# mhsitu/welding_robot

Measured on AMD Instinct MI355X. Metric: acs_generations_per_sec, higher is better.
Workload: dtype f32

## Files before the change

### include/weldacs.h

```cpp
#ifndef WELDACS_H
#define WELDACS_H
#include <stddef.h>
#include <stdint.h>

#ifdef __cplusplus
extern "C" {
#endif

typedef enum {
    WA_OK = 0,
    WA_ERR_ARG = 1,
    WA_ERR_DEVICE = 2,
    WA_ERR_ALLOC = 3,
    WA_ERR_FILE = 4,
    WA_ERR_FORMAT = 5,
    WA_ERR_POINT = 6,
    WA_ERR_CAPACITY = 7,
    WA_ERR_STATE = 8
} wa_status;

typedef struct wa_ctx wa_ctx;
typedef struct wa_grid wa_grid;
typedef struct wa_acs wa_acs;
typedef struct wa_traj wa_traj;
// ... 78 lines not shown
int wa_acs_read_pheromone(wa_acs *s, int32_t slot, float *out );
int wa_acs_read_ants(wa_acs *s, int32_t slot, int32_t *colony, float *L, int32_t *len, int32_t cap);
int wa_acs_read_ant_path(wa_acs *s, int32_t slot, int32_t ant, int32_t *ids, int32_t cap, int32_t *len);
int wa_acs_last_params(wa_acs *s, int32_t slot, int32_t *colony, float *lambda, float *Q);

enum { WA_K_WALK = 0, WA_K_RANK = 1, WA_K_EVAPORATE = 2, WA_K_DEPOSIT = 3, WA_K_COUNT = 4 };
int wa_acs_profile(wa_acs *s, int32_t enable, int32_t sample_every);
int wa_acs_walk_info(const wa_acs *s, int32_t out[4]);
int wa_acs_profile_read(wa_acs *s, double ms[WA_K_COUNT], int64_t launches[WA_K_COUNT]);
int wa_acs_debug_counters(wa_acs *s, uint64_t out16[16], int32_t reset);
int wa_acs_straggler_counters(wa_acs *s, int32_t slot, uint64_t *handed_over, uint64_t *resumed, int32_t reset);
int wa_acs_set_stragglers(wa_acs *s, int32_t generations);
int wa_acs_converged_info(wa_acs *s, int32_t slot, uint64_t out[4]);
int wa_acs_converged_host_info(wa_acs *s, uint64_t out[4]);
int wa_acs_converged_owed_info(wa_acs *s, uint64_t out[5]);
int wa_acs_evaporate(wa_acs *s, int32_t slot, float rho, int32_t repeats);

#define WA_COMM_ID_BYTES 128
typedef struct wa_comm wa_comm;
int wa_comm_unique_id(uint8_t id_out[WA_COMM_ID_BYTES]);
int wa_comm_create(wa_ctx *ctx, int32_t rank, int32_t world, const uint8_t id[WA_COMM_ID_BYTES], wa_comm **out);
void wa_comm_destroy(wa_comm *c);
int wa_comm_info(const wa_comm *c, int32_t *rank, int32_t *world);
int wa_comm_abort(wa_comm *c);
int wa_comm_stats(wa_comm *c, int64_t out[5]);
int wa_acs_allreduce_best(wa_acs *s, wa_comm *c, int32_t gen0, int32_t count);
int wa_comm_read_best(wa_comm *c, int32_t gen0, int32_t count, float *out);
int wa_comm_read_best_owner(wa_comm *c, int32_t gen0, int32_t count, float *cost, int32_t *owner_rank, int32_t *owner_slot);
int wa_comm_pack_best_key(float cost, int32_t rank, int32_t slot, uint64_t *key);
int wa_comm_unpack_best_key(uint64_t key, float *cost, int32_t *rank, int32_t *slot);
// ... 289 lines not shown
```

### welding_robot_amd/_lib.py

```python
import ctypes as C
import os

HERE = os.path.dirname(os.path.abspath(__file__))
LIB_PATH = os.environ.get("WELDACS_LIB") or os.path.join(HERE, "lib", "libweldacs.so")

WA_OK = 0
STATUS = {0: "WA_OK", 1: "WA_ERR_ARG", 2: "WA_ERR_DEVICE", 3: "WA_ERR_ALLOC", 4: "WA_ERR_FILE",
          5: "WA_ERR_FORMAT", 6: "WA_ERR_POINT", 7: "WA_ERR_CAPACITY", 8: "WA_ERR_STATE"}
RNG_REF, RNG_DEV = 0, 1
K_WALK, K_RANK, K_EVAPORATE, K_DEPOSIT, K_COUNT = 0, 1, 2, 3, 4


class AcsParams(C.Structure):
    _fields_ = [("alpha", C.c_int32), ("beta", C.c_float), ("rho", C.c_float), ("pheromone_0", C.c_float),
                ("max_iteration", C.c_int32), ("predict", C.c_float), ("fixed_colony", C.c_int32),
                ("rng_mode", C.c_int32), ("seed", C.c_uint64)]


class GtspParams(C.Structure):
    _fields_ = [("rng_mode", C.c_int32), ("seed", C.c_uint64), ("stream", C.c_uint32),
                ("max_iterations", C.c_int32)]


WA_D2_NONE = 0x7fffffff
# ... 153 lines not shown
    "wa_acs_result_batch": (C.c_int, [_V, _I, _P, _P, _P, _I64]),
    "wa_acs_result_batch_choices": (C.c_int, [_V, _I, _P, _P, _P, _P, _I64]),
    "wa_acs_trace": (C.c_int, [_V, _I, _P, _P, _P, _P, _P, _P]),
    "wa_acs_export_trace": (C.c_int, [_V, _V, _I, _I]),
    "wa_acs_read_pheromone": (C.c_int, [_V, _I, _P]),
    "wa_acs_read_ants": (C.c_int, [_V, _I, _P, _P, _P, _I]),
    "wa_acs_read_ant_path": (C.c_int, [_V, _I, _I, _P, _I, _P]),
    "wa_acs_last_params": (C.c_int, [_V, _I, _P, _P, _P]),
    "wa_acs_profile": (C.c_int, [_V, _I, _I]),
    "wa_acs_profile_read": (C.c_int, [_V, _P, _P]),
    "wa_acs_debug_counters": (C.c_int, [_V, _P, _I]),
    "wa_acs_straggler_counters": (C.c_int, [_V, _I, _P, _P, _I]),
    "wa_acs_converged_info": (C.c_int, [_V, _I, _P]),
    "wa_acs_converged_host_info": (C.c_int, [_V, _P]),
    "wa_acs_converged_owed_info": (C.c_int, [_V, _P]),
    "wa_acs_set_stragglers": (C.c_int, [_V, _I]),
    "wa_acs_walk_info": (C.c_int, [_V, _P]),
    "wa_acs_evaporate": (C.c_int, [_V, _I, _F, _I]),
    "wa_comm_unique_id": (C.c_int, [_P]),
    "wa_comm_create": (C.c_int, [_V, _I, _I, _P, C.POINTER(_V)]),
    "wa_comm_destroy": (None, [_V]),
    "wa_comm_info": (C.c_int, [_V, _P, _P]),
    "wa_comm_abort": (C.c_int, [_V]),
    "wa_comm_stats": (C.c_int, [_V, _P]),
    "wa_acs_allreduce_best": (C.c_int, [_V, _V, _I, _I]),
    "wa_comm_read_best": (C.c_int, [_V, _I, _I, _P]),
    "wa_comm_read_best_owner": (C.c_int, [_V, _I, _I, _P, _P, _P]),
    "wa_comm_pack_best_key": (C.c_int, [_F, _I, _I, _P]),
    "wa_comm_unpack_best_key": (C.c_int, [C.c_uint64, _P, _P, _P]),
    "wa_comm_allgather_costs": (C.c_int, [_V, _I, _P, _P, _I, _P]),
# ... 95 lines not shown
```

### welding_robot_amd/api.py

```python
import atexit
import ctypes as C
import weakref

import numpy as np

from . import _lib as L
from ._lib import AcsParams, GtspParams, RNG_DEV, RNG_REF, WA_COST_MAX, WA_D2_NONE, WA_DIST_NONE, WA_HOPS_NONE, WeldacsError


RETIME_Q = 1 << 30


def _ptr(a):
    return a.ctypes.data if a is not None else None


_live_contexts = weakref.WeakSet()


@atexit.register
def _close_live_contexts():
    for c in list(_live_contexts):
        try:
            c.close()
# ... 500 lines not shown

    def converged_info(self, slot=0):
        out = (C.c_uint64 * 4)()
        self.ctx.check(self.ctx.lib.wa_acs_converged_info(self.h, slot, out))
        return dict(enqueued=int(out[0]), whole=int(out[1]), cut=int(out[2]), generations=int(out[3]))

    def converged_host_info(self):
        out = (C.c_uint64 * 4)()
        self.ctx.check(self.ctx.lib.wa_acs_converged_host_info(self.h, out))
        return [int(v) for v in out]

    def converged_owed_info(self):
        out = (C.c_uint64 * 5)()
        self.ctx.check(self.ctx.lib.wa_acs_converged_owed_info(self.h, out))
        return dict(carried=int(out[0]), merged=int(out[1]), fallback=int(out[2]), out_of_place=int(out[3]), in_place=int(out[4]))

    def set_stragglers(self, generations):
        self.ctx.check(self.ctx.lib.wa_acs_set_stragglers(self.h, generations))

    def set_pipeline(self, groups):
        self.ctx.check(self.ctx.lib.wa_acs_set_pipeline(self.h, groups))

    def pipeline_groups(self):
        g = C.c_int32()
        self.ctx.check(self.ctx.lib.wa_acs_pipeline_info(self.h, C.byref(g)))
        return g.value

    def solve(self, params, starts, ends, streams=None):
        starts, ends, streams = self._arrs(starts, ends, streams)
        self.n_active = len(starts)
# ... 661 lines not shown
```

### welding_robot_amd/csrc/acs_converged.hpp

```cpp
#pragma once

#define WA_CONV_CHECK_WAVES 4
#define WA_CONV_ADV_WAVES 4
#define WA_CONV_THREADS ((WA_CONV_CHECK_WAVES + WA_CONV_ADV_WAVES) * 64)
#define WA_CONV_BLOCKS 64
#define WA_CONV_BLOCKS_MAX 256
#define WA_CONV_MAX_WINDOW 64
#define WA_CONV_NODE_CAP 1024
#define WA_CONV_NODE_LDS 128
#define WA_CONV_SNAP 14

struct WaConvHdr {
    uint32_t rem;
    uint32_t ticket;
    int32_t pending;
    int32_t carried;
    unsigned long long whole, cut, gens;
    unsigned long long pad2_[3];
};
static_assert(WA_CONV_SNAP == 14, "wa_table_rows strides the owed records by 14 floats");
static_assert(sizeof(WaConvHdr) == 64, "the snapshots start 64 bytes into the block");

__device__ __forceinline__ WaConvHdr *wa_conv_hdr(const WaAcsDev &D, int32_t slot) { return reinterpret_cast<WaConvHdr *>(D.conv + (int64_t)slot * D.conv_stride); }
__device__ __forceinline__ float *wa_conv_snap(const WaAcsDev &D, int32_t slot, int32_t t)
{
    return reinterpret_cast<float *>(D.conv + (int64_t)slot * D.conv_stride + sizeof(WaConvHdr)) + (int64_t)t * D.conv_nodes * WA_CONV_SNAP;
}
__device__ __forceinline__ int32_t wa_conv_pending(const WaAcsDev &D, int32_t slot) { return wa_conv_hdr(D, slot)->pending; }
__device__ __forceinline__ bool wa_conv_carried(const WaAcsDev &D, int32_t slot) { return wa_conv_hdr(D, slot)->carried != 0; }
__device__ __forceinline__ const float *wa_conv_owed_records(const WaAcsDev &D, int32_t slot) { return wa_conv_snap(D, slot, wa_conv_pending(D, slot) - 1); }
#define WA_CONV_CARRIED 0x80u

__device__ __forceinline__ void wa_conv_flush_rows(const WaAcsDev &D, int32_t slot, int32_t first, int32_t step, bool rows_only)
{
    const int32_t blen = D.ctl[slot].best_len, j = wa_conv_pending(D, slot);
    if (j < 1) return;
    const float *snap = wa_conv_snap(D, slot, j - 1);
    const int32_t *bpath = D.bestpath + (int64_t)slot * D.path_cap;
    float *pher = D.pher + (int64_t)slot * D.pher_stride;
    float *T = D.rtab + (int64_t)slot * D.path_cap * 8;
    for (int32_t x = first; x < blen * WA_CONV_SNAP; x += step) {
        const int32_t i = x / WA_CONV_SNAP, q = x - i * WA_CONV_SNAP;
        const float v = snap[x];
        if (q < 6) { if (!rows_only) pher[(int64_t)(bpath[i] & (int32_t)WA_ID_MASK) * 6 + q] = v; }
// ... 264 lines not shown
```

### welding_robot_amd/csrc/acs_dev.hpp

```cpp
#pragma once

#define WA_GEN_SPEC 0x40000000
#define WA_GEN_OWED 0x20000000
#define WA_GEN_FLAGS (WA_GEN_SPEC | WA_GEN_OWED)

struct WaAcsDev {
    WaDims d;
    const float *cx, *cy, *cz;
    const uint8_t *occ;
    float *pher, *heur;
    unsigned long long *mask;
    uint8_t *mask8;
    uint32_t *bestmark;
    int32_t *bestpos;
    uint8_t *besttabu;
    int32_t *bestpath;
    float *rtab;
    int32_t *paths;
    float *antL;
    int32_t *antLen;
    int32_t *antRep;
    int32_t *perm;
    float *depA;
    float *sortk;
// ... 230 lines not shown
```

### welding_robot_amd/csrc/acs_update.hpp

```cpp
#pragma once
struct WaRec { float k; int32_t t; };
__device__ inline void ss_push_heap(WaRec *first, long hole, long top, WaRec value)
{
    long parent = (hole - 1) / 2;
    while (hole > top && first[parent].k < value.k) {
        first[hole] = first[parent];
        hole = parent;
        parent = (hole - 1) / 2;
    }
    first[hole] = value;
}
__device__ inline void ss_adjust_heap(WaRec *first, long hole, long len, WaRec value)
{
    const long top = hole;
    long child = hole;
    while (child < (len - 1) / 2) {
        child = 2 * (child + 1);
        if (first[child].k < first[child - 1].k) child--;
        first[hole] = first[child];
        hole = child;
    }
    if ((len & 1) == 0 && child == (len - 2) / 2) {
        child = 2 * (child + 1);
        first[hole] = first[child - 1];
// ... 203 lines not shown
        c.bestL = bestL;
        c.dep_lambda = lambda;
        c.dep_Q = Q;
        c.dep_bestL = bestL;
        c.n_dep = s_ndep;
        c.gen = gen + 1;
        c.rep_mask = 0;
        wa_next_params(c, R, (gen + 1) & 1);
        *ctl = c;
    }
}

typedef float wa_v4f __attribute__((ext_vector_type(4)));
__device__ __forceinline__ int32_t wa_conv_pending(const WaAcsDev &D, int32_t slot);
__device__ __forceinline__ bool wa_conv_carried(const WaAcsDev &D, int32_t slot);
template <int NT>
__device__ __forceinline__ wa_v4f wa_sweep_ld(const wa_v4f *p) { return (NT & 1) ? __builtin_nontemporal_load(p) : *p; }
template <int NT>
__device__ __forceinline__ void wa_sweep_st(wa_v4f *p, wa_v4f v)
{
    if (NT & 2) __builtin_nontemporal_store(v, p);
    else *p = v;
}
template <int NT>
__device__ __forceinline__ void wa_sweep_body_nt(const float *src, float *dst, int64_t n_floats, float rho, int32_t ebx, int32_t E, int32_t reps)
{
    const wa_v4f *s4 = reinterpret_cast<const wa_v4f *>(src);
    wa_v4f *d4 = reinterpret_cast<wa_v4f *>(dst);
    const int64_t n4 = n_floats >> 2;
    const int64_t gsz = (int64_t)E * blockDim.x;
// ... 24 lines not shown
    default: wa_sweep_body_nt<3>(src, dst, n_floats, rho, ebx, E, reps); break;
    }
}

#define WA_LEN_OF(x) ((x) & 0x3fffffff)
template <bool SPARSE, int NB>
__global__ __launch_bounds__(256) void k_evap_rank_mark(WaAcsDev D, WaRun R, const float *src_base,
                                                        float *dst_base, int32_t E, int32_t gen, int32_t MB, int32_t split_log2, int32_t lazy_period,
                                                        int32_t sweep_nt, int32_t rank_cap)
{
    extern __shared__ unsigned long long wa_rank_lds[];
    const int32_t slot = blockIdx.y, tid = threadIdx.x;
    const int32_t gflags = gen & WA_GEN_FLAGS;
    gen &= ~WA_GEN_FLAGS;
    if ((gflags & WA_GEN_SPEC) && gen + 1 != D.ctl[slot].spec_until) return;
    if (gen < D.ctl[slot].spec_until) {
        if (!SPARSE && NB == 6 && gen + 1 == D.ctl[slot].spec_until && (int32_t)blockIdx.x >= MB) {
            if ((gflags & WA_GEN_OWED) && wa_conv_carried(D, slot)) return;
            const int32_t j = wa_conv_pending(D, slot);
            float *to = dst_base + (int64_t)slot * D.pher_stride;
            wa_sweep_body((j & 1) ? src_base + (int64_t)slot * D.pher_stride : to, to, (int64_t)NB * D.d.n, R.rho, (int32_t)blockIdx.x - MB, E, sweep_nt, j);
        }
        return;
    }
    if ((int32_t)blockIdx.x >= MB) {
#ifdef WA_TEST_KNOBS
        if (sweep_nt & 0x100) return;
#endif
        if (!SPARSE) {
            float *to = dst_base + (int64_t)slot * D.pher_stride;
// ... 453 lines not shown
```

### welding_robot_amd/csrc/acs_walk.hpp

```cpp
#pragma once
struct WaTabu {
    int32_t *tab;
    uint32_t mask, shift;
    uint32_t *bits;
    bool spilled;
    bool t16 = false;
    uint32_t kmul = 0;
    int32_t hl = 0;
    int32_t ovf_dw = 0;
};
#define WA_T16_EMPTY 0xFFFFu
#define WA_T16_SENTINEL 0xFFFEu
#define WA_T16_MAXD 13u
__device__ __forceinline__ uint32_t wa_t16_idx(const WaTabu &t, uint32_t tt) { return tt >> (32 - t.hl); }
__device__ __forceinline__ uint32_t wa_t16_cmp(const WaTabu &t, uint32_t tt) { return (tt >> (16 - t.hl)) & 0xFFF0u; }
__device__ __forceinline__ bool tabu_has(const WaTabu &t, int32_t key)
{
    if (t.spilled) {
        uint32_t w = __hip_atomic_load(&t.bits[(uint32_t)key >> 5], __ATOMIC_RELAXED, __HIP_MEMORY_SCOPE_AGENT);
        return (w >> (key & 31)) & 1u;
    }
    if (t.t16) {
        const volatile uint16_t *tb = reinterpret_cast<const volatile uint16_t *>(t.tab);
        const uint32_t tt = (uint32_t)key * t.kmul, c = wa_t16_cmp(t, tt);
// ... 848 lines not shown
        if (k2 == 0) T[(int64_t)i * 8 + 7] = __int_as_float(i + 1 < blen ? (int32_t)((uint32_t)wn >> WA_K_SHIFT) : -1);
    }
}

__global__ __launch_bounds__(256) void k_replay_table(WaAcsDev D, WaRun R)
{
    const int32_t row0 = (blockIdx.x * blockDim.x + threadIdx.x) >> 4;
    const int32_t *bpath = D.bestpath + (int64_t)blockIdx.y * D.path_cap;
    const int32_t w0 = row0 < D.path_cap ? bpath[row0] : 0, w1 = row0 + 1 < D.path_cap ? bpath[row0 + 1] : 0;
    wa_table_rows(D, R, blockIdx.y, row0, (gridDim.x * blockDim.x) >> 4, false, 0.f, 0, w0, w1);
}

#define WA_TABLE_BLOCKS_MAX 64
__device__ __forceinline__ void wa_conv_flush_rows(const WaAcsDev &D, int32_t slot, int32_t first, int32_t step, bool rows_only);
__device__ __forceinline__ bool wa_conv_carried(const WaAcsDev &D, int32_t slot);
__device__ __forceinline__ const float *wa_conv_owed_records(const WaAcsDev &D, int32_t slot);
__global__ __launch_bounds__(256) void k_apply_table(WaAcsDev D, WaRun R, int32_t split_log2, int32_t table_blocks, int32_t gen)
{
    const int32_t slot = blockIdx.y;
    const int32_t spec_until = D.ctl[slot].spec_until;
    const int32_t gflags = gen & WA_GEN_FLAGS;
    gen &= ~WA_GEN_FLAGS;
    if ((gflags & WA_GEN_SPEC) && gen + 1 != spec_until) return;
    if (gen + 1 < spec_until) return;
    if (D.dcount && blockIdx.x == 0 && threadIdx.x == 0) D.dcount[slot * 2] = D.dcount[slot * 2 + 1];
    if (D.pool_n && blockIdx.x == 0) {
        const WaStrag sg = wa_strag_of(D, slot);
        sg.arr_len[threadIdx.x] = 0xffffffffu;
        if (threadIdx.x == 0) { *sg.arr_n = 0; sg.pool_n[D.ctl[slot].gen & 1] = 0; }
    }
    if (gen < spec_until) {
        if ((int32_t)blockIdx.x < table_blocks)
            wa_conv_flush_rows(D, slot, blockIdx.x * blockDim.x + threadIdx.x, table_blocks * blockDim.x, (gflags & WA_GEN_OWED) && wa_conv_carried(D, slot));
        return;
    }
    if ((int32_t)blockIdx.x < table_blocks) {
        const int32_t lane = threadIdx.x & 63, row0 = (blockIdx.x * blockDim.x + threadIdx.x) >> 4;
        const float dep_lane = lane < D.max_colony ? D.depA[(int64_t)slot * D.max_colony + lane] : 0.f;
// ... 2 lines not shown
        const int32_t n_dep = D.ctl[slot].n_dep;
        wa_table_rows(D, R, slot, row0, (table_blocks * blockDim.x) >> 4, true, dep_lane, n_dep < 64 ? n_dep : 64, w0, w1,
                      (gflags & WA_GEN_OWED) ? wa_conv_owed_records(D, slot) : nullptr);
        return;
    }
    const int32_t ab = (int32_t)blockIdx.x - table_blocks;
    wa_apply_body<6>(D, slot, 0, ab >> split_log2, ab & ((1 << split_log2) - 1), 1 << split_log2, true);
}

template <bool ALPHA1, bool SPARSE, bool WARM = true, bool REJ = true, bool DIRECT = false, bool T16 = false>
__global__ __launch_bounds__(64) void k_walk_dev(WaAcsDev D, WaRun R, int hash_log2, int32_t gen, int32_t walk_flags)
{
    extern __shared__ int32_t lds[];
    const int32_t slot = blockIdx.y, ant = blockIdx.x;
    const WaSlotCtl *c = &D.ctl[slot];
    if (gen < c->spec_until) return;
    const int32_t colony = c->colony[gen & 1];
#ifdef WA_STRAG_TIME
    if (threadIdx.x == 0 && gen < 128) atomicMax(&wa_strag_t[gen * 8 + 0], ~(unsigned long long)wall_clock64());
#endif
    if (!SPARSE && ALPHA1 && D.pool_n && (int32_t)blockIdx.x >= D.max_colony) {
        const int32_t r = (int32_t)blockIdx.x - D.max_colony, pg = (gen - 1) & 1;
        const WaStrag sg = wa_strag_of(D, slot);
        if (gen < 1 || r >= sg.pool_n[pg] || r >= WA_RESUME_MAX) return;
        const int32_t a = sg.pool_rec[(pg * WA_RESUME_MAX + r) * WA_POOL_REC], n0 = sg.pool_rec[(pg * WA_RESUME_MAX + r) * WA_POOL_REC + 1];
        WaAcsDev Dp = D;
        Dp.pher = const_cast<float *>(D.prev_pher);
        const uint64_t key = wa_ctr_antkey(wa_ctr_key(R.seed, c->stream, (uint32_t)(gen - 1)), (uint32_t)a);
        int32_t f0 = 0, b0 = 0, rs0 = 0;
        wa_walk_one<1, true, false, WARM, false, DIRECT, T16>(Dp, R, slot, a, c->start, c->end, key, lds, hash_log2, rs0, f0, b0, &D.ctl[slot].flags, 0, INFINITY, 0.f, 0u,
// ... 175 lines not shown
```

### welding_robot_amd/csrc/host_acs.inc

```
static int acs_drain(wa_acs *s);
void wa_acs_default_params(wa_acs_params *p)
{
    if (!p) return;
    p->alpha = 1;
    p->beta = 0.6f;
    p->rho = 0.8f;
    p->pheromone_0 = 1.f;
    p->max_iteration = 150;
    p->predict = 10.f;
    p->fixed_colony = 0;
    p->rng_mode = WA_RNG_DEV;
    p->seed = 1;
}


static_assert(WA_PLAN_REF_SPEC_LEN == WA_REF_SPEC_LEN && WA_PLAN_REF_SUPER == WA_REF_SUPER && WA_PLAN_RESUME_MAX == WA_RESUME_MAX &&
              WA_PLAN_POOL_REC == WA_POOL_REC && WA_PLAN_ROW26 == WA_ROW26, "acs_plan.hpp and the kernels' headers disagree");
static WaPlanIn acs_plan_in(const wa_grid *grid, int32_t n_slots, int32_t max_colony, int64_t path_capacity, int32_t nb, bool lazy)
{
    int32_t fields0 = n_slots < 4 ? n_slots : 4;
    if (n_slots >= 32) fields0 = n_slots / 8 < 8 ? 8 : (n_slots / 8 > 24 ? 24 : n_slots / 8);
    return WaPlanIn{grid->d.n, grid->d.nxy, n_slots, max_colony, fields0, path_capacity, nb, lazy ? 1 : 0,
                    env_int("WA_MASK_U64", 0), env_int("WA_REPLAY", 1), env_int("WA_REF_SPEC", 1), env_int("WA_STRAGGLERS", 1), env_int("WA_STRAGGLER_SLOTS", 16),
                    (int64_t)sizeof(WaSlotCtl), (int64_t)sizeof(WaGlibcRand)};
// ... 107 lines not shown
    s->hw_queues = env_int("GPU_MAX_HW_QUEUES", 4);
    s->drain_ok = env_int("WA_STRAGGLER_DRAIN", 1) != 0;
    s->sweep_nt_env = env_int("WA_SWEEP_NT", -1);
    s->straggler_gens = env_int("WA_STRAGGLER_GENS", 64);
    s->conv_on = env_int("WA_CONVERGED_RUN", 1) != 0;
    s->conv_window = env_int("WA_CONVERGED_WINDOW", 32);
    if (s->conv_window > WA_CONV_MAX_WINDOW) s->conv_window = WA_CONV_MAX_WINDOW;
    if (s->conv_window < 1) s->conv_on = false;
    s->conv_nodes_env = env_int("WA_CONVERGED_NODES", 0);
    s->conv_blocks = env_int("WA_CONVERGED_BLOCKS", WA_CONV_BLOCKS);
    s->conv_blocks = s->conv_blocks < 1 ? 1 : s->conv_blocks > WA_CONV_BLOCKS_MAX ? WA_CONV_BLOCKS_MAX : s->conv_blocks;
    s->conv_readback = env_int("WA_CONVERGED_READBACK", 1) != 0;
    s->conv_wait_us = env_int("WA_CONVERGED_WAIT_US", 200000);
    s->conv_spec = env_int("WA_CONVERGED_SPECULATE", 1) != 0;
    s->conv_owed = env_int("WA_CONVERGED_OWED", 1) != 0;
    s->conv_enqueued.assign((size_t)n_slots, 0);
    {
        const int64_t n4 = (int64_t)nb * n / 4;
        int64_t blocks = n4 <= ((int64_t)8 << 20) ? 4096 : n4 / 555;
        if (blocks > 65536) blocks = 65536;
        s->evap_blocks = env_int("WA_EVAP_BLOCKS", (int)blocks);
    }
    hipError_t e = hipSuccess;
    const bool trace_create = env_int("WA_TRACE_CREATE", 0) != 0;
    const auto t_create0 = std::chrono::steady_clock::now();
    auto since0 = [&]() { return std::chrono::duration<double>(std::chrono::steady_clock::now() - t_create0).count(); };
    bool pools = P.pools;
    for (const WaPlanRow &r : P.rows) {
        if (e || (r.pool && !pools)) continue;
        if (&r == &P.rows[P.heur_row]) { e = (hipError_t)heur_pool_grow(s, &D, (int32_t)P.fields0); continue; }
// ... 338 lines not shown
            else k_heuristic<6><<<hg, 256, 0, ctx->stream>>>(s->D, R.beta, s->d_hlist, s->d_hends);
        }
        he_ = hipGetLastError();
    }
    he_ = he_ ? he_ : hipStreamSynchronize(ctx->stream);
    if (he_ != hipSuccess) {
        for (int32_t f : hlist) { s->heur_end[f] = -1; s->heur_used[f] = 0; }
        s->begun = false;
        return fail(ctx, WA_ERR_DEVICE, "wa_acs_begin: %s", hipGetErrorString(he_));
    }
    s->n_active = n_problems;
    s->begun = true;
    s->gens_enqueued = 0;
    s->conv_until = 0;
    s->conv_prev_whole = false;
    s->conv_owed_flush = s->conv_owed_gen = -1;
    s->ran_before = false;
    return WA_OK;
}

static EvPair *prof_open(wa_acs *s, hipStream_t st, int cls, bool sampled)
{
    if (!sampled) return nullptr;
    EvPair p;
    p.cls = cls;
    if (hipEventCreate(&p.a) != hipSuccess) return nullptr;
    if (hipEventCreate(&p.b) != hipSuccess) { hipEventDestroy(p.a); return nullptr; }
    hipEventRecord(p.a, st);
    s->ev.push_back(p);
    return &s->ev.back();
// ... 137 lines not shown
        if (hipEventCreate(&p.b) == hipSuccess) ev = true;
        else hipEventDestroy(p.a);
    }
    if (ev) {
        if (s->nb == 26) hipExtLaunchKernelGGL((k_evap_rank_mark<false, 26>), grid, dim3(256), rank_lds, G.st, p.a, p.b, 0, G.V, s->R, src, dst, s->evap_blocks, gen, MB, SL, LP, G.sweep_nt, RC);
        else hipExtLaunchKernelGGL((k_evap_rank_mark<false, 6>), grid, dim3(256), rank_lds, G.st, p.a, p.b, 0, G.V, s->R, src, dst, s->evap_blocks, gen, MB, SL, LP, G.sweep_nt, RC);
    } else if (s->nb == 26) {
        k_evap_rank_mark<false, 26><<<grid, 256, rank_lds, G.st>>>(G.V, s->R, src, dst, s->evap_blocks, gen, MB, SL, LP, G.sweep_nt, RC);
    } else {
        k_evap_rank_mark<false, 6><<<grid, 256, rank_lds, G.st>>>(G.V, s->R, src, dst, s->evap_blocks, gen, MB, SL, LP, G.sweep_nt, RC);
    }
    if (ev) s->ev.push_back(p);
}

static void enqueue_generation(wa_acs *s, WaGroupRun &G, int32_t gen, bool last_of_call, bool sampled, bool fused, int32_t chunks,
                               size_t shmem, int32_t P_all, bool owed = false)
{
    wa_ctx *ctx = s->ctx;
    const int32_t P = G.P;
    hipStream_t st = G.st;
    const int64_t off = (int64_t)G.slot0 * s->D.pher_stride;
    float *src = s->pher_buf[G.cur] + off, *dst = s->pher_buf[G.cur ^ (s->lazy ? 0 : 1)] + off;
    G.V.pher = src;
    G.V.prev_pher = s->lazy ? nullptr : s->pher_buf[G.cur ^ 1] + off;
    {
        const int64_t poff = (int64_t)G.slot0 * s->D.max_colony * s->D.path_cap;
        G.V.paths = s->paths_arr[gen & 1] + poff;
        G.V.prev_paths = s->paths_arr[(gen + 1) & 1] + poff;
    }
    EvPair *e = prof_open(s, st, WA_K_WALK, sampled);
    const bool strag = s->D.pool_n != nullptr && fused && s->R.rng_mode == WA_RNG_DEV && s->R.alpha == 1 && gen <= s->straggler_gens;
// ... 12 lines not shown
        }
    } else if (s->R.rng_mode == WA_RNG_DEV) {
        if (s->colony_bound > 0) {
            dim3 wg((unsigned)(strag ? s->D.max_colony + WA_RESUME_MAX : s->colony_bound), (unsigned)P);
            const int walk_flags = s->walk_flags | (hand_over ? 32 : 0);
            const bool warm = s->walk_direct <= 0 && s->tab16_env != 1 && (s->walk_warm < 0 ? (int64_t)s->colony_bound * P_all <= ctx->prop.multiProcessorCount : s->walk_warm != 0);
            const bool rej = (walk_flags & 2) && gen >= ((walk_flags >> 24) & 127);
            const bool direct = !warm && (s->walk_direct < 0 ? walk_direct_rule(s, P_all) : s->walk_direct != 0);
            bool t16 = false;
            if (!warm && !direct && s->R.alpha == 1 && (walk_flags & 1) && s->D.tab16_kmul != 0 && s->id_bits <= s->hash_log2 + 12) {
                int64_t per_cu = 160 * 1024 / (int64_t)shmem;
                if (per_cu > 16) per_cu = 16;
                t16 = s->tab16_env == 1 || (s->tab16_env < 0 && s->id_bits <= 21 && (int64_t)wg.x * P_all > per_cu * ctx->prop.multiProcessorCount);
            }
            const size_t shmem16 = ((size_t)2 << s->hash_log2) + WA_WALK_LDS_EXTRA + (size_t)s->lds_pad;
#define WA_LAUNCH_WALK16(SP, RJ) k_walk_dev<true, SP, false, RJ, false, true><<<wg, 64, shmem16, st>>>(G.V, s->R, s->hash_log2, gen, walk_flags)
#define WA_LAUNCH_WALK(A1, SP, WM, RJ, DR) k_walk_dev<A1, SP, WM, RJ, DR><<<wg, 64, shmem, st>>>(G.V, s->R, s->hash_log2, gen, walk_flags)
            s->last_walk[0] = s->hash_log2; s->last_walk[1] = t16 ? 1 : 0; s->last_walk[2] = (int32_t)(t16 ? shmem16 : shmem); s->last_walk[3] = warm ? 1 : 0;
            if (t16) {
                if (s->lazy) { if (rej) WA_LAUNCH_WALK16(true, true); else WA_LAUNCH_WALK16(true, false); }
                else { if (rej) WA_LAUNCH_WALK16(false, true); else WA_LAUNCH_WALK16(false, false); }
            } else if (s->R.alpha != 1) {
                if (s->lazy) WA_LAUNCH_WALK(false, true, true, true, false); else WA_LAUNCH_WALK(false, false, true, true, false);
            } else if (s->lazy) {
                if (warm) { if (rej) WA_LAUNCH_WALK(true, true, true, true, false); else WA_LAUNCH_WALK(true, true, true, false, false); }
                else if (direct) { if (rej) WA_LAUNCH_WALK(true, true, false, true, true); else WA_LAUNCH_WALK(true, true, false, false, true); }
                else { if (rej) WA_LAUNCH_WALK(true, true, false, true, false); else WA_LAUNCH_WALK(true, true, false, false, false); }
            } else {
                if (warm) { if (rej) WA_LAUNCH_WALK(true, false, true, true, false); else WA_LAUNCH_WALK(true, false, true, false, false); }
                else if (direct) { if (rej) WA_LAUNCH_WALK(true, false, false, true, true); else WA_LAUNCH_WALK(true, false, false, false, true); }
                else { if (rej) WA_LAUNCH_WALK(true, false, false, true, false); else WA_LAUNCH_WALK(true, false, false, false, false); }
            }
// ... 9 lines not shown
        }
        k_walk_ref<<<dim3(1, 1), 64, shmem, st>>>(G.V, s->R, s->hash_log2, gen, (s->walk_flags & 1) | (spec ? 2 : 0));
    }
    prof_close(st, e);
#ifdef WA_STATE_HASH
#define WA_HASH_GENS 256
#define WA_HASH_AT(phase) do { if (s->d_hashlog && gen < WA_HASH_GENS) k_state_hash<<<dim3(96, (unsigned)P), 256, 0, st>>>(G.V, s->R, s->d_hashlog + (((int64_t)gen * 3 + (phase)) * s->n_slots + G.slot0) * 8, (phase)); } while (0)
#else
#define WA_HASH_AT(phase) do { } while (0)
#endif
    WA_HASH_AT(0);
    static const int dbg_sync = env_int("WA_SYNC_DBG", 0);
#define WA_DBG_SYNC(name) do { if (dbg_sync) { fprintf(stderr, "[dbg] %s gen %d slot0 %d P %d ...", name, gen, G.slot0, P); fflush(stderr); hipError_t e_ = hipStreamSynchronize(st); fprintf(stderr, " %s\n", hipGetErrorString(e_)); } } while (0)
    WA_DBG_SYNC("walk");
    if (fused) {
        launch_fused(s, G, src, dst, owed ? gen | WA_GEN_OWED : gen, sampled || s->prof_sweep_all);
        WA_DBG_SYNC("fused sweep+rank+mark");
        if (!s->lazy) G.cur ^= 1;
        G.V.pher = dst;
        WA_HASH_AT(1);
        e = prof_open(s, st, WA_K_DEPOSIT, sampled);
        if (s->nb == 26) k_apply_table26<<<dim3((unsigned)(1 + WA_TABLE26_BLOCKS + mark_blocks(s)), (unsigned)P), 256, 0, st>>>(G.V, s->R);
        else { const int32_t SL = P >= 32 ? 1 : 2, TB = P >= 32 ? 32 : WA_TABLE_BLOCKS_MAX; k_apply_table<<<dim3((unsigned)(TB + ((mark_blocks(s) >> 3) << SL)), (unsigned)P), 256, 0, st>>>(G.V, s->R, SL, TB, owed ? gen | WA_GEN_OWED : gen); }
        prof_close(st, e);
        WA_DBG_SYNC("apply+table");
        WA_HASH_AT(2);
        return;
    }
    e = prof_open(s, st, WA_K_RANK, sampled);
    if (s->nb == 26) k_rank<26><<<P, 256, 0, st>>>(G.V, s->R, gen);
    else k_rank<6><<<P, 256, 0, st>>>(G.V, s->R, gen);
    prof_close(st, e);
    launch_evaporate(s, st, s->pher_buf[G.cur], s->pher_buf[G.cur ^ 1], G.slot0, P, s->R.rho, sampled, G.sweep_nt);
    G.cur ^= 1;
    G.V.pher = dst;
    e = prof_open(s, st, WA_K_DEPOSIT, sampled);
    for (int32_t c = 0; c < chunks; c++) {
        dim3 dg(8, 64, (unsigned)P);
// ... 149 lines not shown
}

static hipError_t enqueue_spec_flush(wa_acs *s, WaGroupRun &G, int32_t gen, int32_t gflags)
{
    const int64_t off = (int64_t)G.slot0 * s->D.pher_stride;
    float *src = s->pher_buf[G.cur] + off, *dst = s->pher_buf[G.cur ^ 1] + off;
    G.V.pher = src;
    G.V.prev_pher = dst;
    launch_fused(s, G, src, dst, gen | gflags, false);
    G.cur ^= 1;
    G.V.pher = dst;
    const int32_t SL = 2, TB = WA_TABLE_BLOCKS_MAX;
    k_apply_table<<<dim3((unsigned)(TB + ((mark_blocks(s) >> 3) << SL)), (unsigned)G.P), 256, 0, G.st>>>(G.V, s->R, SL, TB, gen | gflags);
    return hipGetLastError();
}
static hipError_t enqueue_owed_rows(wa_acs *s, WaGroupRun &G, int32_t gen)
{
    G.cur ^= 1;
    G.V.pher = s->pher_buf[G.cur] + (int64_t)G.slot0 * s->D.pher_stride;
    const int32_t SL = 2, TB = WA_TABLE_BLOCKS_MAX;
    k_apply_table<<<dim3((unsigned)TB, (unsigned)G.P), 256, 0, G.st>>>(G.V, s->R, SL, TB, gen | WA_GEN_OWED);
    return hipGetLastError();
}

int wa_acs_run(wa_acs *s, int32_t n_generations)
{
    WaDevGuard dev_guard_(s ? s->ctx : nullptr);
    if (!dev_guard_.ok) return WA_ERR_DEVICE;
    if (!s || n_generations < 0) return WA_ERR_ARG;
    wa_ctx *ctx = s->ctx;
    if (!s->begun) return fail(ctx, WA_ERR_STATE, "wa_acs_run before wa_acs_begin");
    const int32_t P = s->n_active;
    const size_t shmem = (sizeof(int32_t) << s->hash_log2) + WA_WALK_LDS_EXTRA + (size_t)s->lds_pad;
    if (!ctx->lds_attr_set) {
        const int lds_max = (int)((sizeof(int32_t) << 15) + WA_WALK_LDS_EXTRA);
        hipError_t a = hipSuccess;
// ... 24 lines not shown
    if (n_generations > 0 && s->pending_resume) {
        const bool carries = s->D.pool_n != nullptr && fused && s->R.rng_mode == WA_RNG_DEV && s->R.alpha == 1 && s->gens_enqueued <= s->straggler_gens;
        if (carries) s->pending_resume = false;
        else { int drc_ = acs_drain(s); if (drc_) return drc_; }
    }
#ifdef WA_STATE_HASH
    if (n_generations > 0 && s->gens_enqueued == 0) {
        const size_t bytes = sizeof(unsigned long long) * 256 * 3 * (size_t)s->n_slots * 8;
        if (!s->d_hashlog) HIPC(ctx, hipMalloc((void **)&s->d_hashlog, bytes));
        HIPC(ctx, hipMemsetAsync(s->d_hashlog, 0, bytes, ctx->stream));
    }
#endif
    const bool conv = n_generations > 1 && conv_rule(s, fused) && conv_scratch(s);
    const bool readback = conv && s->conv_readback && s->h_verdict && P == 1;
    const bool owed_on = readback && s->conv_owed;
    const int32_t gen_last = s->gens_enqueued + n_generations - 1;
    const int32_t NG = n_generations > 0 ? pipe_groups(s, P) : 1;
    s->last_groups = NG;
    std::vector<WaGroupRun> groups((size_t)NG);
    if (NG > 1) {
        while ((int32_t)s->gstream.size() < NG - 1) {
            hipStream_t st = nullptr;
            hipEvent_t ev = nullptr;
            HIPC(ctx, hipStreamCreateWithFlags(&st, hipStreamNonBlocking));
            s->gstream.push_back(st);
            HIPC(ctx, hipEventCreateWithFlags(&ev, hipEventDisableTiming));
            s->gjoin.push_back(ev);
        }
        if (!s->gfork) HIPC(ctx, hipEventCreateWithFlags(&s->gfork, hipEventDisableTiming));
        HIPC(ctx, hipEventRecord(s->gfork, ctx->stream));
// ... 33 lines not shown
                s->conv_seq++;
                if (readback && W >= 3) ask = W;
                owe = owed_on && ask && conv_window_at(s, gen + W, gen_last) < 1;
                for (int32_t k = 0; k < NG; k++) {
                    const hipError_t le = launch_converged(s, groups[(size_t)k], gen, W, owe);
                    if (le != hipSuccess) return fail(ctx, WA_ERR_DEVICE, "wa_acs_run: k_converged_run: %s", hipGetErrorString(le));
                }
                s->conv_until = gen + W;
            }
        }
        int32_t known = -2;
        if (ask && s->conv_spec && s->conv_prev_whole && s->conv_wait_us > 0) {
            WaGroupRun &G = groups[0];
            const int cur0 = G.cur;
            G.cur ^= (ask - 1) & 1;
            const hipError_t fe = enqueue_spec_flush(s, G, gen + ask - 1, WA_GEN_SPEC | (owe ? WA_GEN_OWED : 0));
            if (fe != hipSuccess) return fail(ctx, WA_ERR_DEVICE, "wa_acs_run: speculative flush: %s", hipGetErrorString(fe));
            known = conv_verdict(s, G.st, ask);
            if (known < 0) {
                HIPC(ctx, hipStreamSynchronize(G.st));
                const uint32_t v = __atomic_load_n(s->h_verdict, __ATOMIC_ACQUIRE);
                if ((v >> 8) != (s->conv_seq & 0xffffffu) || (int32_t)(v & 0x7fu) > ask) return fail(ctx, WA_ERR_DEVICE, "wa_acs_run: a window ended without its verdict");
                known = (int32_t)(v & 0x7fu);
                s->conv_carried = known == ask && (v & WA_CONV_CARRIED) != 0;
            }
            if (known == ask) {
                s->gens_enqueued += ask;
                s->conv_host[1] += (uint64_t)(ask - 1);
                g += ask - 1;
                if (owe) {
                    if (s->conv_carried) { s->conv_owed_info[0]++; s->conv_owed_gen = gen + ask; s->conv_owed_reps = ask + 1; }
                    else s->conv_owed_info[2]++;
                }
                continue;
            }
            G.cur = cur0;
            s->conv_host[2]++;
            s->conv_prev_whole = false;
        }
        for (int32_t k = 0; k < NG; k++)
            enqueue_generation(s, groups[(size_t)k], gen, g + 1 == n_generations, sampled, fused, chunks, shmem, P, owed);
        s->gens_enqueued++;
        if (ask) {
            const int32_t j = known != -2 ? known : conv_verdict(s, groups[0].st, ask);
            s->conv_prev_whole = j == ask;
            if (owe && j == ask) {
                if (s->conv_carried) { s->conv_owed_info[0]++; s->conv_owed_flush = gen + ask - 1; s->conv_owed_reps = ask + 1; }
                else s->conv_owed_info[2]++;
            }
            for (int32_t t = 2; t < j; t++) {
                groups[0].cur ^= 1;
                s->gens_enqueued++;
                s->conv_host[1]++;
                g++;
            }
        }
    }
    for (int32_t k = 1; k < NG; k++) {
        HIPC(ctx, hipEventRecord(s->gjoin[(size_t)k - 1], groups[(size_t)k].st));
        HIPC(ctx, hipStreamWaitEvent(ctx->stream, s->gjoin[(size_t)k - 1], 0));
// ... 356 lines not shown
            launch_evaporate(s, s->ctx->stream, src, dst, q, 1, q == slot ? rho : 1.0f, s->prof && q == slot, sweep_policy(s, s->n_slots));
        s->cur_buf ^= 1;
        s->D.pher = dst;
    }
    for (int32_t q = 0; q < s->n_slots; q++) s->slot_buf[q] = s->cur_buf;
    HIPC(s->ctx, hipGetLastError());
    return WA_OK;
}

int wa_acs_converged_owed_info(wa_acs *s, uint64_t out[5])
{
    if (!s || !out) return WA_ERR_ARG;
    for (int i = 0; i < 5; i++) out[i] = s->conv_owed_info[i];
    return WA_OK;
}
int wa_acs_converged_host_info(wa_acs *s, uint64_t out[4])
{
    if (!s || !out) return WA_ERR_ARG;
    for (int i = 0; i < 4; i++) out[i] = s->conv_host[i];
    return WA_OK;
}
int wa_acs_converged_info(wa_acs *s, int32_t slot, uint64_t out[4])
{
    WaDevGuard dev_guard_(s ? s->ctx : nullptr);
    if (!dev_guard_.ok) return WA_ERR_DEVICE;
    if (!s || !out || slot < 0 || slot >= s->n_slots) return WA_ERR_ARG;
    wa_ctx *ctx = s->ctx;
    out[0] = s->conv_enqueued[(size_t)slot];
    out[1] = out[2] = out[3] = 0;
    if (!s->d_conv) return WA_OK;
// ... 8 lines not shown
```

### welding_robot_amd/csrc/weldacs.hip

```cpp
#include "../../include/weldacs.h"

#include <hip/hip_runtime.h>
#include <hip/hip_ext.h>
#include <rccl/rccl.h>

#include <float.h>
#include <locale.h>
#include <math.h>
#include <stdio.h>
#include <stdlib.h>
#include <string.h>

#include <algorithm>
#include <chrono>
#include <functional>
#include <memory>
#include <mutex>
#include <thread>
#include <unordered_map>
#include <string>
#include <vector>

#include "acs_kernels.hpp"
#include "grid_kernels.hpp"
// ... 145 lines not shown
    int32_t conv_snaps = 0;
    std::vector<uint64_t> conv_enqueued;
    bool conv_readback = true;
    int32_t conv_wait_us = 200000;
    uint32_t *h_verdict = nullptr;
    uint32_t conv_seq = 0;
    uint64_t conv_host[4] = {0, 0, 0, 0};
    bool conv_spec = true;
    bool conv_owed = true;
    bool conv_carried = false;
    int32_t conv_owed_flush = -1;
    int32_t conv_owed_gen = -1;
    int32_t conv_owed_reps = 0;
    uint64_t conv_owed_info[5] = {0, 0, 0, 0, 0};
    bool conv_prev_whole = false;
};

static int fail(wa_ctx *c, int code, const char *fmt, const char *a = "", const char *b = "")
{
    if (c) {
        char buf[512];
        snprintf(buf, sizeof buf, fmt, a, b);
        c->err = buf;
    }
    return code;
}
#define HIPC(ctx, call)                                                                       \
    do {                                                                                      \
        hipError_t e_ = (call);                                                               \
        if (e_ != hipSuccess) return fail((ctx), WA_ERR_DEVICE, #call ": %s", hipGetErrorString(e_)); \
// ... 558 lines not shown
```

Before: 32460.

## Speculatively enqueue the next generation ahead of the convergence verdict readback

When the previous convergence verdict was whole and carried, the host now enqueues the owed rows flush and the next full generation, tagged with a new AHEAD flag, before waiting on the verdict readback. Device kernels check the AHEAD flag against spec_until and the carried state and exit early if the speculation turns out wrong. The host rolls back its buffer index, resume state and profiling events when the verdict disagrees. This is meant to hide the host round-trip latency of the verdict behind GPU work, at the cost of extra launches and more complex state tracking.

```diff
diff --git a/include/weldacs.h b/include/weldacs.h
--- a/include/weldacs.h
+++ b/include/weldacs.h
@@ -116,6 +116,7 @@
 int wa_acs_converged_info(wa_acs *s, int32_t slot, uint64_t out[4]);
 int wa_acs_converged_host_info(wa_acs *s, uint64_t out[4]);
 int wa_acs_converged_owed_info(wa_acs *s, uint64_t out[5]);
+int wa_acs_converged_ahead_info(wa_acs *s, uint64_t out[3]);
 int wa_acs_evaporate(wa_acs *s, int32_t slot, float rho, int32_t repeats);
 
 #define WA_COMM_ID_BYTES 128
diff --git a/welding_robot_amd/_lib.py b/welding_robot_amd/_lib.py
--- a/welding_robot_amd/_lib.py
+++ b/welding_robot_amd/_lib.py
@@ -191,6 +191,7 @@
     "wa_acs_converged_info": (C.c_int, [_V, _I, _P]),
     "wa_acs_converged_host_info": (C.c_int, [_V, _P]),
     "wa_acs_converged_owed_info": (C.c_int, [_V, _P]),
+    "wa_acs_converged_ahead_info": (C.c_int, [_V, _P]),
     "wa_acs_set_stragglers": (C.c_int, [_V, _I]),
     "wa_acs_walk_info": (C.c_int, [_V, _P]),
     "wa_acs_evaporate": (C.c_int, [_V, _I, _F, _I]),
diff --git a/welding_robot_amd/api.py b/welding_robot_amd/api.py
--- a/welding_robot_amd/api.py
+++ b/welding_robot_amd/api.py
@@ -538,6 +538,11 @@
         out = (C.c_uint64 * 5)()
         self.ctx.check(self.ctx.lib.wa_acs_converged_owed_info(self.h, out))
         return dict(carried=int(out[0]), merged=int(out[1]), fallback=int(out[2]), out_of_place=int(out[3]), in_place=int(out[4]))
+
+    def converged_ahead_info(self):
+        out = (C.c_uint64 * 3)()
+        self.ctx.check(self.ctx.lib.wa_acs_converged_ahead_info(self.h, out))
+        return dict(enqueued=int(out[0]), ran=int(out[1]), cancelled=int(out[2]))
 
     def set_stragglers(self, generations):
         self.ctx.check(self.ctx.lib.wa_acs_set_stragglers(self.h, generations))
diff --git a/welding_robot_amd/csrc/acs_converged.hpp b/welding_robot_amd/csrc/acs_converged.hpp
--- a/welding_robot_amd/csrc/acs_converged.hpp
+++ b/welding_robot_amd/csrc/acs_converged.hpp
@@ -28,6 +28,10 @@
 }
 __device__ __forceinline__ int32_t wa_conv_pending(const WaAcsDev &D, int32_t slot) { return wa_conv_hdr(D, slot)->pending; }
 __device__ __forceinline__ bool wa_conv_carried(const WaAcsDev &D, int32_t slot) { return wa_conv_hdr(D, slot)->carried != 0; }
+__device__ __forceinline__ bool wa_conv_ahead_go(const WaAcsDev &D, int32_t slot, int32_t gen)
+{
+    return D.ctl[slot].spec_until == gen && wa_conv_hdr(D, slot)->carried != 0;
+}
 __device__ __forceinline__ const float *wa_conv_owed_records(const WaAcsDev &D, int32_t slot) { return wa_conv_snap(D, slot, wa_conv_pending(D, slot) - 1); }
 #define WA_CONV_CARRIED 0x80u
 
diff --git a/welding_robot_amd/csrc/acs_dev.hpp b/welding_robot_amd/csrc/acs_dev.hpp
--- a/welding_robot_amd/csrc/acs_dev.hpp
+++ b/welding_robot_amd/csrc/acs_dev.hpp
@@ -2,7 +2,8 @@
 
 #define WA_GEN_SPEC 0x40000000
 #define WA_GEN_OWED 0x20000000
-#define WA_GEN_FLAGS (WA_GEN_SPEC | WA_GEN_OWED)
+#define WA_GEN_AHEAD 0x10000000
+#define WA_GEN_FLAGS (WA_GEN_SPEC | WA_GEN_OWED | WA_GEN_AHEAD)
 
 struct WaAcsDev {
     WaDims d;
diff --git a/welding_robot_amd/csrc/acs_update.hpp b/welding_robot_amd/csrc/acs_update.hpp
--- a/welding_robot_amd/csrc/acs_update.hpp
+++ b/welding_robot_amd/csrc/acs_update.hpp
@@ -241,6 +241,7 @@
 typedef float wa_v4f __attribute__((ext_vector_type(4)));
 __device__ __forceinline__ int32_t wa_conv_pending(const WaAcsDev &D, int32_t slot);
 __device__ __forceinline__ bool wa_conv_carried(const WaAcsDev &D, int32_t slot);
+__device__ __forceinline__ bool wa_conv_ahead_go(const WaAcsDev &D, int32_t slot, int32_t gen);
 template <int NT>
 __device__ __forceinline__ wa_v4f wa_sweep_ld(const wa_v4f *p) { return (NT & 1) ? __builtin_nontemporal_load(p) : *p; }
 template <int NT>
@@ -295,6 +296,7 @@
     const int32_t gflags = gen & WA_GEN_FLAGS;
     gen &= ~WA_GEN_FLAGS;
     if ((gflags & WA_GEN_SPEC) && gen + 1 != D.ctl[slot].spec_until) return;
+    if ((gflags & WA_GEN_AHEAD) && !wa_conv_ahead_go(D, slot, gen)) return;
     if (gen < D.ctl[slot].spec_until) {
         if (!SPARSE && NB == 6 && gen + 1 == D.ctl[slot].spec_until && (int32_t)blockIdx.x >= MB) {
             if ((gflags & WA_GEN_OWED) && wa_conv_carried(D, slot)) return;
diff --git a/welding_robot_amd/csrc/acs_walk.hpp b/welding_robot_amd/csrc/acs_walk.hpp
--- a/welding_robot_amd/csrc/acs_walk.hpp
+++ b/welding_robot_amd/csrc/acs_walk.hpp
@@ -886,6 +886,7 @@
 #define WA_TABLE_BLOCKS_MAX 64
 __device__ __forceinline__ void wa_conv_flush_rows(const WaAcsDev &D, int32_t slot, int32_t first, int32_t step, bool rows_only);
 __device__ __forceinline__ bool wa_conv_carried(const WaAcsDev &D, int32_t slot);
+__device__ __forceinline__ bool wa_conv_ahead_go(const WaAcsDev &D, int32_t slot, int32_t gen);
 __device__ __forceinline__ const float *wa_conv_owed_records(const WaAcsDev &D, int32_t slot);
 __global__ __launch_bounds__(256) void k_apply_table(WaAcsDev D, WaRun R, int32_t split_log2, int32_t table_blocks, int32_t gen)
 {
@@ -894,6 +895,7 @@
     const int32_t gflags = gen & WA_GEN_FLAGS;
     gen &= ~WA_GEN_FLAGS;
     if ((gflags & WA_GEN_SPEC) && gen + 1 != spec_until) return;
+    if ((gflags & WA_GEN_AHEAD) && !wa_conv_ahead_go(D, slot, (gflags & WA_GEN_SPEC) ? gen + 1 : gen)) return;
     if (gen + 1 < spec_until) return;
     if (D.dcount && blockIdx.x == 0 && threadIdx.x == 0) D.dcount[slot * 2] = D.dcount[slot * 2 + 1];
     if (D.pool_n && blockIdx.x == 0) {
@@ -926,6 +928,10 @@
     extern __shared__ int32_t lds[];
     const int32_t slot = blockIdx.y, ant = blockIdx.x;
     const WaSlotCtl *c = &D.ctl[slot];
+    if (gen & WA_GEN_AHEAD) {
+        gen &= ~WA_GEN_AHEAD;
+        if (!wa_conv_ahead_go(D, slot, gen)) return;
+    }
     if (gen < c->spec_until) return;
     const int32_t colony = c->colony[gen & 1];
 #ifdef WA_STRAG_TIME
diff --git a/welding_robot_amd/csrc/host_acs.inc b/welding_robot_amd/csrc/host_acs.inc
--- a/welding_robot_amd/csrc/host_acs.inc
+++ b/welding_robot_amd/csrc/host_acs.inc
@@ -145,6 +145,7 @@
     s->conv_wait_us = env_int("WA_CONVERGED_WAIT_US", 200000);
     s->conv_spec = env_int("WA_CONVERGED_SPECULATE", 1) != 0;
     s->conv_owed = env_int("WA_CONVERGED_OWED", 1) != 0;
+    s->conv_ahead = env_int("WA_CONVERGED_AHEAD", 1) != 0;
     s->conv_enqueued.assign((size_t)n_slots, 0);
     {
         const int64_t n4 = (int64_t)nb * n / 4;
@@ -513,6 +514,7 @@
     s->gens_enqueued = 0;
     s->conv_until = 0;
     s->conv_prev_whole = false;
+    s->conv_ahead_prev = false;
     s->conv_owed_flush = s->conv_owed_gen = -1;
     s->ran_before = false;
     return WA_OK;
@@ -680,7 +682,7 @@
 }
 
 static void enqueue_generation(wa_acs *s, WaGroupRun &G, int32_t gen, bool last_of_call, bool sampled, bool fused, int32_t chunks,
-                               size_t shmem, int32_t P_all, bool owed = false)
+                               size_t shmem, int32_t P_all, bool owed = false, bool ahead = false)
 {
     wa_ctx *ctx = s->ctx;
     const int32_t P = G.P;
@@ -723,8 +725,9 @@
                 t16 = s->tab16_env == 1 || (s->tab16_env < 0 && s->id_bits <= 21 && (int64_t)wg.x * P_all > per_cu * ctx->prop.multiProcessorCount);
             }
             const size_t shmem16 = ((size_t)2 << s->hash_log2) + WA_WALK_LDS_EXTRA + (size_t)s->lds_pad;
-#define WA_LAUNCH_WALK16(SP, RJ) k_walk_dev<true, SP, false, RJ, false, true><<<wg, 64, shmem16, st>>>(G.V, s->R, s->hash_log2, gen, walk_flags)
-#define WA_LAUNCH_WALK(A1, SP, WM, RJ, DR) k_walk_dev<A1, SP, WM, RJ, DR><<<wg, 64, shmem, st>>>(G.V, s->R, s->hash_log2, gen, walk_flags)
+            const int32_t wgen = ahead ? gen | WA_GEN_AHEAD : gen;
+#define WA_LAUNCH_WALK16(SP, RJ) k_walk_dev<true, SP, false, RJ, false, true><<<wg, 64, shmem16, st>>>(G.V, s->R, s->hash_log2, wgen, walk_flags)
+#define WA_LAUNCH_WALK(A1, SP, WM, RJ, DR) k_walk_dev<A1, SP, WM, RJ, DR><<<wg, 64, shmem, st>>>(G.V, s->R, s->hash_log2, wgen, walk_flags)
             s->last_walk[0] = s->hash_log2; s->last_walk[1] = t16 ? 1 : 0; s->last_walk[2] = (int32_t)(t16 ? shmem16 : shmem); s->last_walk[3] = warm ? 1 : 0;
             if (t16) {
                 if (s->lazy) { if (rej) WA_LAUNCH_WALK16(true, true); else WA_LAUNCH_WALK16(true, false); }
@@ -764,14 +767,15 @@
 #define WA_DBG_SYNC(name) do { if (dbg_sync) { fprintf(stderr, "[dbg] %s gen %d slot0 %d P %d ...", name, gen, G.slot0, P); fflush(stderr); hipError_t e_ = hipStreamSynchronize(st); fprintf(stderr, " %s\n", hipGetErrorString(e_)); } } while (0)
     WA_DBG_SYNC("walk");
     if (fused) {
-        launch_fused(s, G, src, dst, owed ? gen | WA_GEN_OWED : gen, sampled || s->prof_sweep_all);
+        const int32_t ugen = gen | (owed ? WA_GEN_OWED : 0) | (ahead ? WA_GEN_AHEAD : 0);
+        launch_fused(s, G, src, dst, ugen, sampled || s->prof_sweep_all);
         WA_DBG_SYNC("fused sweep+rank+mark");
         if (!s->lazy) G.cur ^= 1;
         G.V.pher = dst;
         WA_HASH_AT(1);
         e = prof_open(s, st, WA_K_DEPOSIT, sampled);
         if (s->nb == 26) k_apply_table26<<<dim3((unsigned)(1 + WA_TABLE26_BLOCKS + mark_blocks(s)), (unsigned)P), 256, 0, st>>>(G.V, s->R);
-        else { const int32_t SL = P >= 32 ? 1 : 2, TB = P >= 32 ? 32 : WA_TABLE_BLOCKS_MAX; k_apply_table<<<dim3((unsigned)(TB + ((mark_blocks(s) >> 3) << SL)), (unsigned)P), 256, 0, st>>>(G.V, s->R, SL, TB, owed ? gen | WA_GEN_OWED : gen); }
+        else { const int32_t SL = P >= 32 ? 1 : 2, TB = P >= 32 ? 32 : WA_TABLE_BLOCKS_MAX; k_apply_table<<<dim3((unsigned)(TB + ((mark_blocks(s) >> 3) << SL)), (unsigned)P), 256, 0, st>>>(G.V, s->R, SL, TB, ugen); }
         prof_close(st, e);
         WA_DBG_SYNC("apply+table");
         WA_HASH_AT(2);
@@ -951,12 +955,12 @@
     k_apply_table<<<dim3((unsigned)(TB + ((mark_blocks(s) >> 3) << SL)), (unsigned)G.P), 256, 0, G.st>>>(G.V, s->R, SL, TB, gen | gflags);
     return hipGetLastError();
 }
-static hipError_t enqueue_owed_rows(wa_acs *s, WaGroupRun &G, int32_t gen)
+static hipError_t enqueue_owed_rows(wa_acs *s, WaGroupRun &G, int32_t gen, int32_t gflags = 0)
 {
     G.cur ^= 1;
     G.V.pher = s->pher_buf[G.cur] + (int64_t)G.slot0 * s->D.pher_stride;
     const int32_t SL = 2, TB = WA_TABLE_BLOCKS_MAX;
-    k_apply_table<<<dim3((unsigned)TB, (unsigned)G.P), 256, 0, G.st>>>(G.V, s->R, SL, TB, gen | WA_GEN_OWED);
+    k_apply_table<<<dim3((unsigned)TB, (unsigned)G.P), 256, 0, G.st>>>(G.V, s->R, SL, TB, gen | WA_GEN_OWED | gflags);
     return hipGetLastError();
 }
 
@@ -1011,6 +1015,7 @@
     const bool conv = n_generations > 1 && conv_rule(s, fused) && conv_scratch(s);
     const bool readback = conv && s->conv_readback && s->h_verdict && P == 1;
     const bool owed_on = readback && s->conv_owed;
+    const bool ahead_on = owed_on && s->conv_ahead && s->conv_spec && s->conv_wait_us > 0;
     const int32_t gen_last = s->gens_enqueued + n_generations - 1;
     const int32_t NG = n_generations > 0 ? pipe_groups(s, P) : 1;
     s->last_groups = NG;
@@ -1074,8 +1079,20 @@
             WaGroupRun &G = groups[0];
             const int cur0 = G.cur;
             G.cur ^= (ask - 1) & 1;
-            const hipError_t fe = enqueue_spec_flush(s, G, gen + ask - 1, WA_GEN_SPEC | (owe ? WA_GEN_OWED : 0));
+            const bool ahead = owe && ahead_on && s->conv_ahead_prev;
+            const hipError_t fe = ahead ? enqueue_owed_rows(s, G, gen + ask - 1, WA_GEN_SPEC | WA_GEN_AHEAD)
+                                        : enqueue_spec_flush(s, G, gen + ask - 1, WA_GEN_SPEC | (owe ? WA_GEN_OWED : 0));
             if (fe != hipSuccess) return fail(ctx, WA_ERR_DEVICE, "wa_acs_run: speculative flush: %s", hipGetErrorString(fe));
+            const int cur1 = G.cur;
+            const bool resume1 = s->pending_resume;
+            const size_t ev1 = s->ev.size();
+            if (ahead) {
+                const int32_t ga = gen + ask;
+                enqueue_generation(s, G, ga, ga == gen_last, s->prof && (ga % s->prof_every) == 0, fused, chunks, shmem, P, true, true);
+                const hipError_t ae = hipGetLastError();
+                if (ae != hipSuccess) return fail(ctx, WA_ERR_DEVICE, "wa_acs_run: generation ahead of the verdict: %s", hipGetErrorString(ae));
+                s->conv_ahead_info[0]++;
+            }
             known = conv_verdict(s, G.st, ask);
             if (known < 0) {
                 HIPC(ctx, hipStreamSynchronize(G.st));
@@ -1084,7 +1101,24 @@
                 known = (int32_t)(v & 0x7fu);
                 s->conv_carried = known == ask && (v & WA_CONV_CARRIED) != 0;
             }
-            if (known == ask) {
+            if (owe) s->conv_ahead_prev = known == ask && s->conv_carried;
+            if (ahead && known == ask && s->conv_carried) {
+                s->gens_enqueued += ask + 1;
+                s->conv_host[1] += (uint64_t)(ask - 1);
+                g += ask;
+                s->conv_owed_info[0]++;
+                s->conv_owed_info[1]++;
+                s->conv_owed_info[((ask + 1) & 1) ? 3 : 4]++;
+                s->conv_ahead_info[1]++;
+                continue;
+            }
+            if (ahead) {
+                G.cur = cur1;
+                s->pending_resume = resume1;
+                for (size_t q = ev1; q < s->ev.size(); q++) s->ev[q].cls = -1;
+                s->conv_ahead_info[2]++;
+            }
+            if (known == ask && !ahead) {
                 s->gens_enqueued += ask;
                 s->conv_host[1] += (uint64_t)(ask - 1);
                 g += ask - 1;
@@ -1104,6 +1138,7 @@
         if (ask) {
             const int32_t j = known != -2 ? known : conv_verdict(s, groups[0].st, ask);
             s->conv_prev_whole = j == ask;
+            if (owe && known == -2) s->conv_ahead_prev = j == ask && s->conv_carried;
             if (owe && j == ask) {
                 if (s->conv_carried) { s->conv_owed_info[0]++; s->conv_owed_flush = gen + ask - 1; s->conv_owed_reps = ask + 1; }
                 else s->conv_owed_info[2]++;
@@ -1490,6 +1525,12 @@
     for (int i = 0; i < 5; i++) out[i] = s->conv_owed_info[i];
     return WA_OK;
 }
+int wa_acs_converged_ahead_info(wa_acs *s, uint64_t out[3])
+{
+    if (!s || !out) return WA_ERR_ARG;
+    for (int i = 0; i < 3; i++) out[i] = s->conv_ahead_info[i];
+    return WA_OK;
+}
 int wa_acs_converged_host_info(wa_acs *s, uint64_t out[4])
 {
     if (!s || !out) return WA_ERR_ARG;
diff --git a/welding_robot_amd/csrc/weldacs.hip b/welding_robot_amd/csrc/weldacs.hip
--- a/welding_robot_amd/csrc/weldacs.hip
+++ b/welding_robot_amd/csrc/weldacs.hip
@@ -183,6 +183,9 @@
     int32_t conv_owed_reps = 0;
     uint64_t conv_owed_info[5] = {0, 0, 0, 0, 0};
     bool conv_prev_whole = false;
+    bool conv_ahead = true;
+    bool conv_ahead_prev = false;
+    uint64_t conv_ahead_info[3] = {0, 0, 0};
 };
 
 static int fail(wa_ctx *c, int code, const char *fmt, const char *a = "", const char *b = "")
```

Result: no change. 32740 (median of 6 runs) (+0.9%).
